# MyNiuuu/MOFA-Video

Measured on AMD Instinct MI355X. Metric: denoised frames/sec, 25f 576x1024 SVD+MOFA, 25 steps, higher is better.
Workload: dtype f16; 1 GPU; MOFA-Video-Traj, 25-frame 576x1024, 25 denoise steps + temporal VAE decode (chunk 8), single trajectory hint, SVD-XT UNet + MOFA-Adapter, CFG 1->3, seeded random weights in the reference checkpoint layout; num_frames=25, height=576, width=1024, num_inference_steps=25, decode_chunk_size=8, parallelism=1 GPU, graph_steps=False, output_finite=True

## Files before the change

include/mofa_hip.h:

```cpp
#ifndef MOFA_HIP_H
#define MOFA_HIP_H

#include <stdint.h>

#ifdef __cplusplus
extern "C" {
#endif

typedef void* mofa_stream_t;

#define MOFA_OK 0
#define MOFA_EINVAL (-22)
#define MOFA_ELAUNCH (-5)

int mofa_version(void);

enum { MOFA_MODE_PLAIN = 0, MOFA_MODE_CONV3X3 = 1, MOFA_MODE_CONVT3 = 2 };
enum { MOFA_ACT_NONE = 0, MOFA_ACT_SILU = 1, MOFA_ACT_GEGLU_PAIR = 2, MOFA_ACT_RELU = 3,
       MOFA_ACT_GELU = 4  };

typedef struct mofa_igemm_args {
    const void* x;
    const void* w;
    const float* bias;
// ... 40 lines not shown
int mofa_gn_nparts(int HW, int C);
int mofa_gn_partial_f16(const void* x, float* part, int nframes, int HW, int C, int ldx, mofa_stream_t stream);
int mofa_gn_partial_from_stats(const float* stats, float* part, int nframes, int HW, int C, mofa_stream_t stream);
int mofa_gn_finalize(const float* part, const float* gamma, const float* beta, float* scale, float* shift,
                     int nframes, int HW, int C, int frames_per_stat, float eps, mofa_stream_t stream);
int mofa_gn_reduce(const float* part, double* sums, int nframes, int HW, int C, int frames_per_stat, mofa_stream_t stream);
int mofa_gn_finalize_sums(const double* sums, const float* gamma, const float* beta, float* scale, float* shift,
                          int nframes, int C, int frames_per_stat, double count_per_group, float eps,
                          mofa_stream_t stream);
int mofa_gn_apply_f16(const void* x, const float* part, const float* gamma, const float* beta, void* y,
                      int nframes, int HW, int C, int ldx, int ldy, int frames_per_stat, float eps, int silu,
                      mofa_stream_t stream);
int mofa_gn_apply_gathered_f16(const void* x, const float* part_all, int nentries, double count_per_group,
                               const float* gamma, const float* beta, void* y, int nframes, int HW, int C,
                               int ldx, int ldy, float eps, int silu, mofa_stream_t stream);
int mofa_affine_act_f16(const void* x, const float* scale, const float* shift, void* y,
                        int nframes, int HW, int C, int ldx, int ldy, int silu, mofa_stream_t stream);
int mofa_layernorm_f16(const void* x, const float* gamma, const float* beta, void* y, int M, int C,
                       int ldx, int ldy, float eps, const float* rowvec, int rv_div, int rv_mod,
                       mofa_stream_t stream);

typedef struct mofa_ff320_args {
    const void* x;
    const float* pos;
    const void* w1p;
    const float* b1;
    const void* w2p;
    const float* b2;
    const void* r2;
    void* out;
    void* out_ln;
    const float* ln_gamma;
    const float* ln_beta;
    int32_t M, ldx, ldo, ldr2, ldoln, HW, T;
    float eps, s_acc, s1, s2, ln_eps;
    int32_t reserved[4];
} mofa_ff320_args;
int mofa_ff320_f16(const mofa_ff320_args* a, mofa_stream_t stream);

typedef struct mofa_lin320_args {
    const void* x;
    const void* wp;
    const float* bias;
    const float* rowvec;
    const void* r1;
    void* out;
    int32_t M, N, ldx, ldo, ldr1, norm;
    int32_t rv_div, rv_mul, rv_mod_in, rv_mod_out;
    float eps, s_acc, s1;
    int32_t reserved[3];
} mofa_lin320_args;
int mofa_lin320_f16(const mofa_lin320_args* a, mofa_stream_t stream);

int mofa_axpby_f32(const float* x, float* y, int64_t n, float a, float b, mofa_stream_t stream);
int mofa_resize_nearest_f32(const float* x, float* y, int n, int H, int W, int h, int w, mofa_stream_t stream);
int mofa_mask_blend_f16(const void* a, const void* b, const float* w, void* out, int M, int C, int HW, int lda,
                        int ldb, int ldo, mofa_stream_t stream);
int mofa_matting_blend_f16(const void* warped, const void* matting, const void* logit, void* out, float* mask_out,
                           int M, int C, int ldw, int ldm, int ldl, int ldo, mofa_stream_t stream);
int mofa_subsample_tokens_f16(const void* x, void* y, int n, int H, int W, int s, int C, int ldx, int ldy,
                              mofa_stream_t stream);
int mofa_axpby_f16(const void* x, void* y, int M, int C, int ldx, int ldy, float a, float b, mofa_stream_t stream);
int mofa_axpby_out_f16(const void* x, const void* y, void* out, int M, int C, int ldx, int ldy, int ldo, float a, float b,
                       mofa_stream_t stream);
int mofa_geglu_f16(const void* x, void* out, int M, int Ch, int ldx, int ldo, mofa_stream_t stream);
int mofa_copy2d_f16(const void* src, void* dst, int M, int C, int lds, int ldd, mofa_stream_t stream);
int mofa_silu_f32(const float* x, float* y, int n, mofa_stream_t stream);
int mofa_cast_f32_to_f16(const float* x, void* y, int64_t n, mofa_stream_t stream);
int mofa_cast_f16_to_f32(const void* x, float* y, int64_t n, mofa_stream_t stream);
int mofa_nchw_f32_to_nhwc_f16(const float* x, void* y, int n, int C, int HW, int ldo, float scale,
                              mofa_stream_t stream);
int mofa_nhwc_f16_to_nchw_f32(const void* x, float* y, int n, int C, int HW, int ldx, mofa_stream_t stream);
int mofa_timestep_embedding(const float* t, float* out, int n, int dim, mofa_stream_t stream);

int64_t mofa_softsplat_ws_bytes(int nflows, int H, int W);
int mofa_softsplat_avg_f16(const void* feat, const float* flow, void* out, void* ws,
                           int nflows, int H, int W, int C, int ldf, int ldo, mofa_stream_t stream);
int mofa_softsplat_scatter_f32(const float* in, const float* flow, float* out_sum, int N, int C, int H, int W,
                               mofa_stream_t stream);
int mofa_softsplat_weight_f32(const float* in, const float* metric, float* out, int N, int C, int H, int W, int mode,
                              mofa_stream_t stream);
int mofa_softsplat_normalize_f32(const float* summed, float* out, int N, int C, int H, int W, int eps_mode, mofa_stream_t stream);
typedef struct mofa_softsplat_grad_args {
    const float* grad;
    const float* flow;
    const float* in;
    const float* metric;
    const float* inv;
    const float* glast;
    float* grad_in;
    float* grad_flow;
    float* grad_metric;
    float* partial;
    int32_t N, C, H, W, prep, slices;
    int32_t reserved[4];
} mofa_softsplat_grad_args;
int mofa_softsplat_norm_f32(const float* flow, float* norm, void* ws, int N, int H, int W, mofa_stream_t stream);
int mofa_softsplat_grad_prologue_f32(const float* grad, const float* out, const float* norm, float* inv, float* glast,
                                     int N, int C, int H, int W, int eps_mode, mofa_stream_t stream);
int mofa_softsplat_grad_f32(const mofa_softsplat_grad_args* a, mofa_stream_t stream);
typedef struct mofa_softsplat_gather_args {
    const float* in;
    const float* flow;
    const float* metric;
    float* out;
    float* norm;
// ... 48 lines not shown
```

mofa_video_amd/_build.py:

```python
import os
import subprocess
from concurrent.futures import ThreadPoolExecutor

HERE = os.path.dirname(os.path.abspath(__file__))
CSRC = os.path.join(HERE, "csrc")
LIB = os.path.join(HERE, "libmofa_hip.so")
PROBE_LIB = os.path.join(HERE, "..", "tools", "libmofa_hip_probe.so")
SOURCES = ["igemm.hip", "igemm8.hip", "igemm320.hip", "ff320.hip", "lin320.hip", "attention.hip", "norm.hip", "elementwise.hip", "softsplat.hip", "output.hip",
           "cmp_ops.hip", "frontend.hip"]
HEADERS = [os.path.join(CSRC, "common.h"), os.path.join(CSRC, "igemm_common.h"), os.path.join(CSRC, "igemm_pipe.h"),
           os.path.join(HERE, "..", "include", "mofa_hip.h")]
FLAGS = ["--offload-arch=gfx950", "-O3", "-std=c++17", "-fPIC"]


def _hipcc():
    hipcc = os.environ.get("HIPCC", "/opt/rocm/bin/hipcc")
    return hipcc if os.path.exists(hipcc) else "hipcc"


def build(force=False, verbose=False, probe=False, variant=None, defines=()):
    objdir = os.path.join(HERE, "build", variant or ("probe" if probe else "lib"))
    os.makedirs(objdir, exist_ok=True)
    lib = os.path.join(HERE, "..", "tools", f"libmofa_hip_{variant}.so") if variant else (PROBE_LIB if probe else LIB)
    hdr_t = max(os.path.getmtime(h) for h in HEADERS if os.path.exists(h))
    flags = FLAGS + (["-DMOFA_PROBE"] if probe else []) + [f"-D{d}" for d in defines]
    jobs = []
    for s in SOURCES:
        src, obj = os.path.join(CSRC, s), os.path.join(objdir, s.replace(".hip", ".o"))
        if force or not os.path.exists(obj) or os.path.getmtime(obj) < max(os.path.getmtime(src), hdr_t):
            jobs.append([_hipcc(), *flags, "-c", src, "-o", obj])
    if not jobs and os.path.exists(lib) and all(os.path.getmtime(lib) >= os.path.getmtime(os.path.join(objdir, s.replace(".hip", ".o")))
                                                for s in SOURCES):
        return lib

    def run(cmd):
        if verbose:
            print(" ".join(cmd), flush=True)
        subprocess.run(cmd, check=True)
    with ThreadPoolExecutor(max_workers=min(len(jobs), os.cpu_count() or 4) or 1) as ex:
        list(ex.map(run, jobs))
    run([_hipcc(), "--offload-arch=gfx950", "-shared", "-fPIC", *[os.path.join(objdir, s.replace(".hip", ".o")) for s in SOURCES],
         "-o", lib])
    return lib


if __name__ == "__main__":
    import sys
    var = sys.argv[sys.argv.index("--variant") + 1] if "--variant" in sys.argv else None
    print(build(force="--incremental" not in sys.argv, verbose=True, probe="--probe" in sys.argv, variant=var,
                defines=[a[2:] for a in sys.argv if a.startswith("-D")]))
```

mofa_video_amd/blocks.py:

```python
import math

import torch

from . import lib as L
from . import ops
from .weights import (f32, interleave_geglu, pack_conv3d_t3, pack_conv3x3, pack_ff320, pack_lin320, pack_linear, pad_rows)

BIG = 1 << 30


class Sub:

    def __init__(self, sd, prefix="", device="cuda"):
        self.sd, self.prefix, self.device = sd, prefix, device

    def sub(self, name):
        return Sub(self.sd, f"{self.prefix}{name}.", self.device)

    def has(self, name):
        return f"{self.prefix}{name}" in self.sd

    def get(self, name):
        return self.sd[f"{self.prefix}{name}"].detach()

    def dev(self, t):
        return t.to(self.device)


class Ctx:

    def __init__(self, B, T):
        self.B, self.T = B, T
        self.N = B * T
        self.temb_act = None
        self.temb_all = None
        self.ctx16 = None
        self.cache = {}
        self.time_context_hw_major = True
        self.par = None
        self.ctx16_all = None
        self.half = 0
        self.halves = None


class Linear:
    def __init__(self, s, pad_n=False):
        w = s.get("weight")
        w = w.reshape(w.shape[0], -1)
        self.n_real = w.shape[0]
        b = s.get("bias") if s.has("bias") else None
        if pad_n:
            w = pad_rows(w)
            b = pad_rows(b) if b is not None else None
        self.w = s.dev(pack_linear(w))
        self.b = s.dev(f32(b)) if b is not None else None

    def __call__(self, x, **kw):
        return ops.igemm(x, self.w, self.b, **kw)

# ... 171 lines not shown
            return self.tconv2(g, T, HW, s_acc=1.0 - self.alpha, r1=xs, s1=1.0, stats=out_stats, out=out)
        assert c.B == 1
        g = _sharded_norm_convt3(self.tnorm1, self.tconv1, xs, c, HW,
                                 **(tvec(self.ttemb, self.ttemb_off) if self.ttemb is not None else {}))
        return _sharded_norm_convt3(self.tnorm2, self.tconv2, g, c, HW, s_acc=1.0 - self.alpha, r1=xs, s1=1.0, out=out)


def _sharded_norm_convt3(norm, conv, x, c, HW, r1=None, out=None, **epi):
    par, T = c.par, c.T
    M, Cc = T * HW, x.shape[1]
    nparts = ops.gn_nparts(HW, Cc)
    buf, own = par.part_buffer(nparts, x.device)
    ops.gn_partial_into(x, own, T, HW)
    halo = par.halo_begin(x, HW)
    par.gather_partials(buf, nparts)
    cnt = float(par.T_full) * HW * (Cc // 32)
    ext = torch.empty(((T + 2) * HW, Cc), dtype=x.dtype, device=x.device)
    ops.gn_apply_gathered(x, buf, cnt, norm.g, norm.b, norm.eps, ext[HW:(T + 1) * HW], T, HW, silu=True)
    if out is None:
        out = torch.empty((M, conv.w.shape[0]), dtype=x.dtype, device=x.device)
    geom = ops.convt3_geom(0, HW)

    def launch(f0, f1):
        rr = r1[f0 * HW:f1 * HW] if r1 is not None else None
        ops.igemm(ext[(f0 + 1) * HW:], conv.w, conv.b, geom=geom, M=(f1 - f0) * HW, out=out[f0 * HW:f1 * HW], r1=rr, **epi)
    split = par.split_convs and T >= 4
    if split:
        launch(1, T - 1)
    fp, fn = halo.wait()
    for src, dst in ((fp, ext[:HW]), (fn, ext[(T + 1) * HW:])):
        if src is None:
            dst.zero_()
        else:
            ops.gn_apply_gathered(src, buf, cnt, norm.g, norm.b, norm.eps, dst, 1, HW, silu=True)
    if split:
        launch(0, 1)
        launch(T - 1, T)
    else:
        launch(0, T)
    return out


class CrossAttnVec:

    def __init__(self, s):
        self.to_v = Linear(s.sub("to_v"))
        self.to_out = Linear(s.sub("to_out.0"))

    def __call__(self, ctx16):
        return ops.cast_f16_to_f32(self.to_out(self.to_v(ctx16)))


class SelfAttn:
    def __init__(self, s, heads, fold_q_scale=False, norm=None, norm_eps=1e-5):
        wq = s.get("to_q.weight")
        self.heads = heads
        self.C = wq.shape[0]
        self.head_dim = self.C // heads
        assert self.head_dim in (64, 128), f"unsupported head dim {self.head_dim}"
        self.q_prescaled = bool(fold_q_scale)
        if fold_q_scale:
            wq = (wq.float() * (self.head_dim ** -0.5 * ops.Q_FOLD_LOG2E)).to(wq.dtype)
        w = torch.cat([wq, s.get("to_k.weight"), s.get("to_v.weight")], 0)
        self.wqkv = s.dev(pack_linear(w))
        self.to_out = Linear(s.sub("to_out.0"))
        self.qkv_pk = None
        if norm is not None and self.C == 320:
            wp, bp = pack_lin320(w, None, norm.get("weight"), norm.get("bias"))
            self.qkv_pk = (s.dev(wp), s.dev(bp), norm_eps)

    def qkv_normed(self, x):
        wp, bp, eps = self.qkv_pk
        qkv = ops.lin320(x, wp, bp, norm=True, eps=eps)
        Cc = self.C
        return qkv[:, :Cc], qkv[:, Cc:2 * Cc], qkv[:, 2 * Cc:]

    @property
    def can_fuse_norm(self):
        return self.qkv_pk is not None and ops.LIN320

    def qkv(self, x):
        qkv = ops.igemm(x, self.wqkv)
        Cc = self.C
        return qkv[:, :Cc], qkv[:, Cc:2 * Cc], qkv[:, 2 * Cc:]

    def kv_into(self, x, out):
        return ops.igemm(x, self.wqkv[self.C:], out=out)

    def q(self, x):
        return ops.igemm(x, self.wqkv[:self.C])


class TransformerSpatioTemporal:
    _uid = 0

    def __init__(self, s, heads):
        TransformerSpatioTemporal._uid += 1
        self.uid = TransformerSpatioTemporal._uid
        self.heads = heads
        self.norm = GroupNorm(s.sub("norm"), 1e-6)
        self.proj_in, self.proj_out = Linear(s.sub("proj_in")), Linear(s.sub("proj_out"))
        b = s.sub("transformer_blocks.0")
        self.norm1, self.norm3 = LayerNorm(b.sub("norm1")), LayerNorm(b.sub("norm3"))
        self.attn1, self.attn2, self.ff = (SelfAttn(b.sub("attn1"), heads, fold_q_scale=True, norm=b.sub("norm1")), CrossAttnVec(b.sub("attn2")),
                                           GegluFF(b.sub("ff"), norm=b.sub("norm3")))
        t = s.sub("temporal_transformer_blocks.0")
        self.norm_in, self.tnorm1, self.tnorm3 = LayerNorm(t.sub("norm_in")), LayerNorm(t.sub("norm1")), LayerNorm(t.sub("norm3"))
        self.ff_in, self.tattn1, self.tattn2, self.tff = (GegluFF(t.sub("ff_in"), norm=t.sub("norm_in")), SelfAttn(t.sub("attn1"), heads),
                                                          CrossAttnVec(t.sub("attn2")), GegluFF(t.sub("ff"), norm=t.sub("norm3")))
        self.pos1, self.pos2 = Linear(s.sub("time_pos_embed.linear_1")), Linear(s.sub("time_pos_embed.linear_2"))
        self.alpha = _sigmoid(s.get("time_mixer.mix_factor").reshape(-1)[0])
        self.C = self.proj_in.w.shape[1]

    def _invariants(self, c):
        key = ("xf", self.uid)
        if key not in c.cache:
            dev = self.proj_in.w.device
            f0 = c.par.f0 if c.par is not None else 0
            tpos = ops.timestep_embedding(torch.arange(f0, f0 + c.T, dtype=torch.float32, device=dev), self.C)
            e = self.pos2(self.pos1(ops.cast_f32_to_f16(tpos), act=L.ACT_SILU))
            v_tm = self.tattn2(c.ctx16_all if c.ctx16_all is not None else c.ctx16)
            c.cache[key] = (self.attn2(c.ctx16), v_tm, ops.cast_f16_to_f32(e))
        return c.cache[key]

    def __call__(self, x, c, H, W, out_stats=False, out=None):
        HW, N, T, B = H * W, c.N, c.T, c.B
        v_sp, v_tm, pos = self._invariants(c)
        h = self.norm(x, N, HW)
        h = self.proj_in(h)
        fuse_qkv = self.attn1.can_fuse_norm and ops.lin320_fits(h.shape[0], 3 * self.C)
        q, k, v = self.attn1.qkv_normed(h) if fuse_qkv else self.attn1.qkv(self.norm1(h))
        a = ops.attn_spatial(q, k, v, N, self.heads, HW, head_dim=self.attn1.head_dim, prescaled=self.attn1.q_prescaled)
        h = self.attn1.to_out(a, r1=h, s1=1.0, rowvec=v_sp, rv=(T * HW, 1, 1, BIG))
        h = self.ff.fused(h) if self.ff.can_fuse else self.ff(self.norm3(h), r1=h, s1=1.0)
        pos_rv = (HW, 1, 1, T)
        fn = None
        if self.ff_in.can_fuse:
            f_own = None
            if c.par is not None and c.par.kv_slots <= 32 and c.par.kv_inplace and c.par.gather_hidden:
                hid, f_own = c.par.kv_buffer(HW, self.C, h.device)
            f, fn = self.ff_in.fused(h, pos=pos, HW=HW, T=T, ln_out=(self.tnorm1.g, self.tnorm1.b, f_own), ln_eps=self.tnorm1.eps)
        else:
            f = self.ff_in(self.norm_in(h, rowvec=pos, rv_div=HW, rv_mod=T), r1=h, s1=1.0, rowvec=pos, rv=pos_rv)
        if c.par is None:
            q, k, v = self.tattn1.qkv(fn if fn is not None else self.tnorm1(f))
            a = ops.attn_temporal(q, k, v, B, T, HW, self.heads, head_dim=self.tattn1.head_dim)
        else:
            Cc, par = self.C, c.par
            if par.kv_slots <= 32 and par.kv_inplace and par.gather_hidden:
                if fn is None:
                    hid, own = par.kv_buffer(HW, Cc, f.device)
                    fn = self.tnorm1(f, out=own)
                work = par.kv_gather_begin(hid, HW)
                q = self.tattn1.q(fn)
                work.wait()
                kv = ops.igemm(hid, self.tattn1.wqkv[Cc:])
                a = ops.attn_temporal(q, kv[:, :Cc], kv[:, Cc:], 1, par.kv_slots, HW, self.heads,
                                      head_dim=self.tattn1.head_dim, Tq=T, key_mask=par.kv_mask)
            elif par.kv_slots <= 32 and par.kv_inplace:
                fn = fn if fn is not None else self.tnorm1(f)
                kv, own = par.kv_buffer(HW, 2 * Cc, fn.device)
                self.tattn1.kv_into(fn, own)
                work = par.kv_gather_begin(kv, HW)
                q = self.tattn1.q(fn)
                work.wait()
                a = ops.attn_temporal(q, kv[:, :Cc], kv[:, Cc:], 1, par.kv_slots, HW, self.heads,
                                      head_dim=self.tattn1.head_dim, Tq=T, key_mask=par.kv_mask)
            else:
                fn = fn if fn is not None else self.tnorm1(f)
                q, k, v = self.tattn1.qkv(fn)
                kv = torch.empty((q.shape[0], 2 * Cc), dtype=torch.float16, device=q.device)
                ops.copy2d(k, kv[:, :Cc])
                ops.copy2d(v, kv[:, Cc:])
                kv = par.gather_frames(kv, HW)
                a = ops.attn_temporal(q, kv[:, :Cc], kv[:, Cc:], 1, par.T_full, HW, self.heads,
                                      head_dim=self.tattn1.head_dim, Tq=T)
        Bg = v_tm.shape[0]
        if not c.time_context_hw_major:
            quirk, tab = (T * HW, 1, 1, BIG), (v_tm if Bg == B else v_tm[c.half:c.half + B].contiguous())
        elif Bg == B:
            quirk, tab = (T * HW, HW, HW, B), v_tm
        else:
            rot = (c.half * HW) % Bg
            tab = torch.cat([v_tm[rot:], v_tm[:rot]], 0).contiguous() if rot else v_tm
            quirk = (T * HW, 0, HW, Bg)
        f = self.tattn1.to_out(a, r1=f, s1=1.0, rowvec=tab, rv=quirk)
        al = self.alpha
        if self.tff.can_fuse:
            m = self.tff.fused(f, s_acc=1.0 - al, s1=1.0 - al, r2=h, s2=al)
        else:
            m = self.tff(self.tnorm3(f), s_acc=1.0 - al, r1=f, s1=1.0 - al, r2=h, s2=al)
        return self.proj_out(m, r1=x, s1=1.0, stats=out_stats, out=out)


class DownBlock:
    def __init__(self, s, num_layers, heads, cross, downsample):
        eps = 1e-6 if cross else 1e-5
        self.resnets = [SpatioTemporalResBlock(s.sub(f"resnets.{i}"), eps) for i in range(num_layers)]
        self.attns = [TransformerSpatioTemporal(s.sub(f"attentions.{i}"), heads) for i in range(num_layers)] if cross else None
# ... 92 lines not shown
```

mofa_video_amd/lib.py:

```python
import ctypes as C
import os

import torch

_HERE = os.path.dirname(os.path.abspath(__file__))
LIB_PATH = os.environ.get("MOFA_HIP_LIB") or os.path.join(_HERE, "libmofa_hip.so")

MODE_PLAIN, MODE_CONV3X3, MODE_CONVT3 = 0, 1, 2
ACT_NONE, ACT_SILU, ACT_GEGLU_PAIR, ACT_RELU, ACT_GELU = 0, 1, 2, 3, 4
PAD_SAME, PAD_TRAILING = 0, 1
TILE_AUTO, TILE_128X128, TILE_192X128, TILE_256X256, TILE_256X320 = 0, 2, 4, 5, 6


class IgemmArgs(C.Structure):
    _fields_ = [
        ("x", C.c_void_p), ("w", C.c_void_p), ("bias", C.c_void_p), ("rowvec", C.c_void_p),
        ("r1", C.c_void_p), ("r2", C.c_void_p), ("out", C.c_void_p),
        ("M", C.c_int32), ("N", C.c_int32), ("Cin", C.c_int32),
        ("ldx", C.c_int32), ("ldo", C.c_int32), ("ldr1", C.c_int32), ("ldr2", C.c_int32),
        ("mode", C.c_int32),
        ("Hin", C.c_int32), ("Win", C.c_int32), ("Hout", C.c_int32), ("Wout", C.c_int32),
        ("stride", C.c_int32), ("up", C.c_int32), ("ksize", C.c_int32),
        ("T", C.c_int32), ("HW", C.c_int32),
        ("rv_div", C.c_int32), ("rv_mul", C.c_int32), ("rv_mod_in", C.c_int32), ("rv_mod_out", C.c_int32),
        ("act", C.c_int32),
        ("s_acc", C.c_float), ("s1", C.c_float), ("s2", C.c_float),
        ("dil", C.c_int32), ("pad", C.c_int32), ("tile", C.c_int32),
        ("workspace", C.c_void_p), ("workspace_bytes", C.c_int64),
        ("stats", C.c_void_p),
    ]


class Ff320Args(C.Structure):
    _fields_ = [
        ("x", C.c_void_p), ("pos", C.c_void_p), ("w1p", C.c_void_p), ("b1", C.c_void_p), ("w2p", C.c_void_p), ("b2", C.c_void_p),
        ("r2", C.c_void_p), ("out", C.c_void_p), ("out_ln", C.c_void_p), ("ln_gamma", C.c_void_p), ("ln_beta", C.c_void_p),
        ("M", C.c_int32), ("ldx", C.c_int32), ("ldo", C.c_int32), ("ldr2", C.c_int32), ("ldoln", C.c_int32),
        ("HW", C.c_int32), ("T", C.c_int32),
        ("eps", C.c_float), ("s_acc", C.c_float), ("s1", C.c_float), ("s2", C.c_float), ("ln_eps", C.c_float),
        ("reserved", C.c_int32 * 4),
    ]


class Lin320Args(C.Structure):
    _fields_ = [
        ("x", C.c_void_p), ("wp", C.c_void_p), ("bias", C.c_void_p), ("rowvec", C.c_void_p), ("r1", C.c_void_p), ("out", C.c_void_p),
        ("M", C.c_int32), ("N", C.c_int32), ("ldx", C.c_int32), ("ldo", C.c_int32), ("ldr1", C.c_int32), ("norm", C.c_int32),
        ("rv_div", C.c_int32), ("rv_mul", C.c_int32), ("rv_mod_in", C.c_int32), ("rv_mod_out", C.c_int32),
        ("eps", C.c_float), ("s_acc", C.c_float), ("s1", C.c_float),
        ("reserved", C.c_int32 * 3),
    ]


class SoftsplatGradArgs(C.Structure):
    _fields_ = [
        ("grad", C.c_void_p), ("flow", C.c_void_p), ("inp", C.c_void_p), ("metric", C.c_void_p), ("inv", C.c_void_p),
        ("glast", C.c_void_p), ("grad_in", C.c_void_p), ("grad_flow", C.c_void_p), ("grad_metric", C.c_void_p),
        ("partial", C.c_void_p),
        ("N", C.c_int32), ("C", C.c_int32), ("H", C.c_int32), ("W", C.c_int32), ("prep", C.c_int32), ("slices", C.c_int32),
        ("reserved", C.c_int32 * 4),
    ]


class SoftsplatGatherArgs(C.Structure):
    _fields_ = [
        ("inp", C.c_void_p), ("flow", C.c_void_p), ("metric", C.c_void_p), ("out", C.c_void_p), ("norm", C.c_void_p), ("ws", C.c_void_p),
        ("N", C.c_int32), ("C", C.c_int32), ("H", C.c_int32), ("W", C.c_int32), ("prep", C.c_int32), ("normalize", C.c_int32),
        ("eps_mode", C.c_int32), ("slices", C.c_int32),
        ("reserved", C.c_int32 * 4),
    ]


_P, _I, _F, _L = C.c_void_p, C.c_int, C.c_float, C.c_int64

PROTOTYPES = {
    "mofa_version": [],
    "mofa_igemm_f16": [_P, _P],
    "mofa_igemm_stats_ok": [_P],
    "mofa_ff320_f16": [_P, _P],
    "mofa_lin320_f16": [_P, _P],
    "mofa_attn_spatial_f16": [_P, _P, _P, _P, _I, _I, _I, _I, _I, _I, _I, _I, _F, _P],
    "mofa_attn_spatial_qb_f16": [_P, _P, _P, _P, _I, _I, _I, _I, _I, _I, _I, _I, _F, _I, _P],
    "mofa_transpose_v_f16": [_P, _P, _I, _I, _I, _I, _P],
    "mofa_attn_temporal_f16": [_P, _P, _P, _P, _I, _I, _I, _I, _I, _I, _I, _I, _I, _F, _P],
    "mofa_attn_temporal_masked_f16": [_P, _P, _P, _P, _I, _I, _I, _I, _I, _I, _I, _I, _I, _F, C.c_uint32, _P],
    "mofa_softmax_rows_f16": [_P, _I, _I, _I, _P],
    "mofa_gn_nparts": [_I, _I],
    "mofa_gn_partial_f16": [_P, _P, _I, _I, _I, _I, _P],
    "mofa_gn_partial_from_stats": [_P, _P, _I, _I, _I, _P],
    "mofa_gn_finalize": [_P, _P, _P, _P, _P, _I, _I, _I, _I, _F, _P],
    "mofa_gn_reduce": [_P, _P, _I, _I, _I, _I, _P],
    "mofa_gn_finalize_sums": [_P, _P, _P, _P, _P, _I, _I, _I, C.c_double, _F, _P],
    "mofa_gn_apply_f16": [_P, _P, _P, _P, _P, _I, _I, _I, _I, _I, _I, _F, _I, _P],
    "mofa_gn_apply_gathered_f16": [_P, _P, _I, C.c_double, _P, _P, _P, _I, _I, _I, _I, _I, _F, _I, _P],
    "mofa_affine_act_f16": [_P, _P, _P, _P, _I, _I, _I, _I, _I, _I, _P],
    "mofa_layernorm_f16": [_P, _P, _P, _P, _I, _I, _I, _I, _F, _P, _I, _I, _P],
    "mofa_axpby_f32": [_P, _P, _L, _F, _F, _P],
    "mofa_resize_nearest_f32": [_P, _P, _I, _I, _I, _I, _I, _P],
    "mofa_mask_blend_f16": [_P, _P, _P, _P, _I, _I, _I, _I, _I, _I, _P],
    "mofa_matting_blend_f16": [_P, _P, _P, _P, _P, _I, _I, _I, _I, _I, _I, _P],
    "mofa_subsample_tokens_f16": [_P, _P, _I, _I, _I, _I, _I, _I, _I, _P],
    "mofa_axpby_f16": [_P, _P, _I, _I, _I, _I, _F, _F, _P],
    "mofa_axpby_out_f16": [_P, _P, _P, _I, _I, _I, _I, _I, _F, _F, _P],
    "mofa_geglu_f16": [_P, _P, _I, _I, _I, _I, _P],
    "mofa_copy2d_f16": [_P, _P, _I, _I, _I, _I, _P],
    "mofa_silu_f32": [_P, _P, _I, _P],
    "mofa_cast_f32_to_f16": [_P, _P, _L, _P],
    "mofa_cast_f16_to_f32": [_P, _P, _L, _P],
    "mofa_nchw_f32_to_nhwc_f16": [_P, _P, _I, _I, _I, _I, _F, _P],
    "mofa_nhwc_f16_to_nchw_f32": [_P, _P, _I, _I, _I, _I, _P],
    "mofa_timestep_embedding": [_P, _P, _I, _I, _P],
    "mofa_softsplat_ws_bytes": [_I, _I, _I],
    "mofa_softsplat_avg_f16": [_P, _P, _P, _P, _I, _I, _I, _I, _I, _I, _P],
    "mofa_softsplat_scatter_f32": [_P, _P, _P, _I, _I, _I, _I, _P],
    "mofa_softsplat_weight_f32": [_P, _P, _P, _I, _I, _I, _I, _I, _P],
    "mofa_softsplat_normalize_f32": [_P, _P, _I, _I, _I, _I, _I, _P],
    "mofa_softsplat_norm_f32": [_P, _P, _P, _I, _I, _I, _P],
    "mofa_softsplat_grad_prologue_f32": [_P, _P, _P, _P, _P, _I, _I, _I, _I, _I, _P],
    "mofa_softsplat_grad_f32": [_P, _P],
    "mofa_softsplat_gather_f32": [_P, _P],
    "mofa_flow_downscale_f32": [_P, _P, _I, _I, _I, _I, _P],
    "mofa_prepare_model_input": [_P, _P, _P, _I, _I, _I, _F, _P],
    "mofa_cfg_euler_step": [_P, _P, _I, _I, _I, _F, _F, _F, _F, _P],
    "mofa_prepare_model_input_dev": [_P, _P, _P, _I, _I, _I, _P, _P],
    "mofa_cfg_euler_step_dev": [_P, _P, _I, _I, _I, _P, _F, _F, _P],
    "mofa_step_select": [_P, _P, _P, _I, _P],
    "mofa_pool2d_f16": [_P, _P, _I, _I, _I, _I, _I, _I, _I, _I, _I, _I, _P],
    "mofa_resize_bilinear_ac_f16": [_P, _P, _I, _I, _I, _I, _I, _I, _I, _I, _P],
    "mofa_resize_bilinear_ac_f32": [_P, _P, _I, _I, _I, _I, _I, _P],
    "mofa_flow_expectation_f16": [_P, _P, _I, _I, _I, _I, _F, _P],
    "mofa_filter1d_reflect_f32": [_P, _P, _P, _I, _I, _I, _I, _I, _P],
    "mofa_resize_bicubic_ac_f32": [_P, _P, _I, _I, _I, _I, _I, _P],
    "mofa_patchify_f16": [_P, _P, _I, _I, _I, _I, _I, _I, _P],
# ... 42 lines not shown
```

mofa_video_amd/ops.py:

```python
import ctypes as C
import struct
import threading

import torch

from . import lib as L

F16 = torch.float16
F32 = torch.float32


class LaunchTimer:

    def __init__(self):
        self.rec = []
        self.tags = []

    def start(self):
        e = torch.cuda.Event(enable_timing=True)
        e.record()
        return e

    def stop(self, name, e0, flops=0.0, nbytes=0.0, tag=None):
        e1 = torch.cuda.Event(enable_timing=True)
        e1.record()
        self.rec.append((name, e0, e1, flops, nbytes))
        if tag is not None:
            self.tags.append((tag, len(self.rec) - 1))

    def by_tag(self):
        torch.cuda.synchronize()
        out = {}
        for tag, i in self.tags:
            _, e0, e1, fl, _ = self.rec[i]
            d = out.setdefault(tag, [0, 0.0, 0.0])
            d[0] += 1
            d[1] += e0.elapsed_time(e1) * 1e-3
            d[2] += fl
        return out

    def summary(self):
        torch.cuda.synchronize()
        out = {}
        for name, e0, e1, fl, nb in self.rec:
            d = out.setdefault(name, dict(launches=0, seconds=0.0, flops=0.0, bytes=0.0))
            d["launches"] += 1
            d["seconds"] += e0.elapsed_time(e1) * 1e-3
            d["flops"] += fl
            d["bytes"] += nb
        return out


TIMER = None
# ... 250 lines not shown
        _written(yl)
    args = _FF320_ARGS.pack(x.data_ptr(), L.ptr(pos) or 0, w1p.data_ptr(), b1.data_ptr(), w2p.data_ptr(), b2.data_ptr(),
                            L.ptr(r2) or 0, out.data_ptr(), L.ptr(yl) or 0, L.ptr(pg) or 0, L.ptr(pb) or 0,
                            M, _ld(x), _ld(out), _ld(r2) if r2 is not None else 0, _ld(yl) if yl is not None else 0, HW, T,
                            eps, s_acc, s1, s2 if r2 is not None else 0.0, ln_eps, 0, 0, 0, 0)
    t0 = TIMER.start() if TIMER is not None else None
    rc = lib.mofa_ff320_f16(args, L.stream_ptr())
    if rc != 0:
        L.check(rc, "mofa_ff320_f16")
    if t0 is not None:
        TIMER.stop("igemm_f16_kernel", t0, flops=2.0 * M * (2560 * 320 + 320 * 1280), tag=(9, 0, 0, M, 320, 320, 0))
    return out if ln_out is None else (out, yl)


_LIN320_ARGS = struct.Struct("@6P10i3f3i")
assert _LIN320_ARGS.size == C.sizeof(L.Lin320Args)
LIN320 = True


def lin320_fits(M, ldo):
    return (M + 256) * ldo * 2 < 0xFFFFFFFF


def lin320(x, wp, bias=None, norm=False, eps=1e-5, rowvec=None, rv=(1, 1, 1, 1 << 30), r1=None, s1=1.0, s_acc=1.0, out=None):
    lib = L.load()
    _chk(x, F16)
    M, N = x.shape[0], wp.shape[0] * 64
    assert x.shape[1] == 320 and wp.dtype is F16 and wp.numel() == N * 320
    if out is None:
        out = torch.empty((M, N), dtype=F16, device=x.device)
    else:
        assert out.dtype is F16 and out.shape[0] == M and out.shape[1] >= N
        _written(out)
    if bias is not None:
        assert bias.dtype is F32 and bias.numel() == N
    if rowvec is not None:
        assert rowvec.dtype is F32 and rowvec.dim() == 2 and rowvec.shape[1] == N and rowvec.stride(1) == 1
        assert rowvec.is_contiguous() or (rowvec.stride(0) % N == 0 and rv[1] == rowvec.stride(0) // N), (rowvec.stride(), N, rv)
    if r1 is not None:
        assert r1.dtype is F16 and r1.shape[0] == M and r1.shape[1] >= N
    args = _LIN320_ARGS.pack(x.data_ptr(), wp.data_ptr(), L.ptr(bias) or 0, L.ptr(rowvec) or 0, L.ptr(r1) or 0, out.data_ptr(),
                             M, N, _ld(x), _ld(out), _ld(r1) if r1 is not None else 0, 1 if norm else 0,
                             rv[0], rv[1], rv[2], rv[3], eps, s_acc, s1, 0, 0, 0)
    t0 = TIMER.start() if TIMER is not None else None
    rc = lib.mofa_lin320_f16(args, L.stream_ptr())
    if rc != 0:
        L.check(rc, "mofa_lin320_f16")
    if t0 is not None:
        TIMER.stop("igemm_f16_kernel", t0, flops=2.0 * M * N * 320, tag=(10, 0, 0, M, N, 320, 0))
    return out


Q_FOLD_LOG2E = 1.4426950408889634


def attn_spatial(q, k, v, nframes, heads, S, head_dim=64, scale=None, out=None, prescaled=False, query_blocks=0):
    lib = L.load()
    Cc = heads * head_dim
    scale = -1.0 if prescaled else (head_dim ** -0.5 if scale is None else scale)
    st = L.stream_ptr()
    if out is None:
        out = torch.empty((nframes * S, Cc), dtype=F16, device=q.device)
    else:
        _written(out)
    t0 = TIMER.start() if TIMER is not None else None
    L.check(lib.mofa_attn_spatial_qb_f16(L.ptr(q), L.ptr(k), L.ptr(v), L.ptr(out), nframes, heads, head_dim, S, _ld(q),
                                         _ld(k), _ld(v), _ld(out), scale, int(query_blocks), st), "mofa_attn_spatial_qb_f16")
    if t0 is not None:
        TIMER.stop("attn_spatial_kernel", t0, flops=4.0 * S * S * Cc * nframes)
    return out


def attn_temporal(q, k, v, nclips, T, HW, heads, head_dim=64, scale=None, out=None, Tq=None, key_mask=None):
    lib = L.load()
    assert _ld(k) == _ld(v)
    Tq = T if Tq is None else Tq
    scale = head_dim ** -0.5 if scale is None else scale
    if out is None:
        out = torch.empty((nclips * Tq * HW, heads * head_dim), dtype=F16, device=q.device)
    else:
        _written(out)
    if key_mask is None:
        L.check(lib.mofa_attn_temporal_f16(L.ptr(q), L.ptr(k), L.ptr(v), L.ptr(out), nclips, Tq, T, HW, heads, head_dim,
                                           _ld(q), _ld(k), _ld(out), scale, L.stream_ptr()), "mofa_attn_temporal_f16")
    else:
        L.check(lib.mofa_attn_temporal_masked_f16(L.ptr(q), L.ptr(k), L.ptr(v), L.ptr(out), nclips, Tq, T, HW, heads, head_dim,
                                                  _ld(q), _ld(k), _ld(out), scale, int(key_mask), L.stream_ptr()),
                "mofa_attn_temporal_masked_f16")
    return out


def softmax_rows_(x):
    lib = L.load()
    L.check(lib.mofa_softmax_rows_f16(L.ptr(x), x.shape[0], x.shape[1], _ld(x), L.stream_ptr()), "mofa_softmax_rows_f16")
    return x


def transpose_v(v, nframes, ncb, S):
    lib = L.load()
    vt = torch.empty((nframes * ncb * 64, S), dtype=F16, device=v.device)
    L.check(lib.mofa_transpose_v_f16(L.ptr(v), L.ptr(vt), nframes, ncb, S, _ld(v), L.stream_ptr()),
            "mofa_transpose_v_f16")
    return vt


def axpby_(x, y, a=1.0, b=1.0):
# ... 443 lines not shown
```

mofa_video_amd/weights.py:

```python
import torch

KPAD = 64


def _pad_cin(w, dim):
    cin = w.shape[dim]
    pad = (-cin) % KPAD
    if pad == 0:
        return w
    shape = list(w.shape)
    shape[dim] = pad
    return torch.cat([w, w.new_zeros(shape)], dim=dim)


def pack_linear(w):
    w = w.reshape(w.shape[0], -1)
    return _pad_cin(w, 1).to(torch.float16).contiguous()


def pack_conv3x3(w):
    w = _pad_cin(w, 1)
    n, cin, kh, kw = w.shape
    return w.permute(0, 2, 3, 1).reshape(n, kh * kw * cin).to(torch.float16).contiguous()

# ... 8 lines not shown
    pad = (-w.shape[0]) % mult
    if pad == 0:
        return w
    return torch.cat([w, w.new_zeros((pad,) + tuple(w.shape[1:]))], dim=0)


def interleave_geglu(w, b):
    n2 = w.shape[0]
    ch = n2 // 2
    assert ch % 16 == 0
    idx = torch.arange(n2).reshape(2, ch // 16, 16).permute(1, 0, 2).reshape(-1)
    return w[idx].contiguous(), (b[idx].contiguous() if b is not None else None)


def pack_ff320(w1, b1, w2, gamma, beta):
    C, H = 320, 1280
    w1, w2 = w1.detach().float().cpu().reshape(2 * H, C), w2.detach().float().cpu().reshape(C, H)
    gamma, beta = gamma.detach().float().cpu(), beta.detach().float().cpu()
    b1f = (b1.detach().float().cpu() if b1 is not None else torch.zeros(2 * H)) + w1 @ beta
    w1g = (w1 * gamma[None, :]).to(torch.float16)
    lane = torch.arange(64)
    n, lh = lane % 32, lane // 32
    c, t, s_, e = torch.arange(40), torch.arange(2), torch.arange(20), torch.arange(8)
    rows = (t[None, :, None, None, None] * H + 32 * c[:, None, None, None, None] + n[None, None, None, :, None])
    cols = 16 * s_[None, None, :, None, None] + 8 * lh[None, None, None, :, None] + e[None, None, None, None, :]
    w1p = w1g[rows.expand(40, 2, 20, 64, 8), cols.expand(40, 2, 20, 64, 8)].contiguous()
    j, u, jj = torch.arange(10), torch.arange(2), torch.arange(8)
    rows2 = 32 * j[None, :, None, None, None] + n[None, None, None, :, None]
    cols2 = (32 * c[:, None, None, None, None] + 16 * u[None, None, :, None, None] + 4 * lh[None, None, None, :, None] +
             (jj & 3)[None, None, None, None, :] + 8 * (jj >> 2)[None, None, None, None, :])
    w2p = w2.to(torch.float16)[rows2.expand(40, 10, 2, 64, 8), cols2.expand(40, 10, 2, 64, 8)].contiguous()
    return w1p, b1f.contiguous(), w2p


def pack_lin320(w, b=None, gamma=None, beta=None):
    w = w.detach().float().cpu().reshape(w.shape[0], -1)
    N, K = w.shape
    assert K == 320 and N % 64 == 0, (N, K)
    bias = b.detach().float().cpu().clone() if b is not None else None
    if beta is not None:
        bias = (bias if bias is not None else torch.zeros(N)) + w @ beta.detach().float().cpu()
    if gamma is not None:
        w = w * gamma.detach().float().cpu()[None, :]
    wh = w.to(torch.float16)
    lane = torch.arange(64)
    n, lh = lane % 32, lane // 32
    c, t, s_, e = torch.arange(N // 64), torch.arange(2), torch.arange(20), torch.arange(8)
    rows = 64 * c[:, None, None, None, None] + 32 * t[None, :, None, None, None] + n[None, None, None, :, None]
    cols = 16 * s_[None, None, :, None, None] + 8 * lh[None, None, None, :, None] + e[None, None, None, None, :]
    shp = (N // 64, 2, 20, 64, 8)
    return wh[rows.expand(shp), cols.expand(shp)].contiguous(), (bias.contiguous() if bias is not None else None)


def f32(t):
    return t.detach().to(torch.float32).contiguous()
```

Baseline: 4.197 frames/s.

## Fuse QKV projection and temporal attention into one kernel for C=320

Adds a HIP kernel that, for the 320-channel temporal self-attention, computes per-head Q, K and V projections with MFMA from weights streamed into LDS, runs softmax attention over the T frames in registers, and writes the output directly. It replaces the separate QKV GEMM and temporal attention launch, so the QKV intermediate never goes through global memory. Weights are repacked per head (q,k,v interleaved) at load time, and the kernel is persistent with a rotating three-slot DMA buffer. It is only used for C=320, 5 heads, T<=32, and is on by default but can be disabled through an environment variable.

```diff
diff --git a/include/mofa_hip.h b/include/mofa_hip.h
--- a/include/mofa_hip.h
+++ b/include/mofa_hip.h
@@ -116,6 +116,16 @@
 } mofa_lin320_args;
 int mofa_lin320_f16(const mofa_lin320_args* a, mofa_stream_t stream);
 
+typedef struct mofa_tattn320_args {
+    const void* x;
+    const void* wp;
+    void* out;
+    int32_t nclips, T, HW, ldx, ldo;
+    float scale;
+    int32_t reserved[4];
+} mofa_tattn320_args;
+int mofa_tattn320_f16(const mofa_tattn320_args* a, mofa_stream_t stream);
+
 int mofa_axpby_f32(const float* x, float* y, int64_t n, float a, float b, mofa_stream_t stream);
 int mofa_resize_nearest_f32(const float* x, float* y, int n, int H, int W, int h, int w, mofa_stream_t stream);
 int mofa_mask_blend_f16(const void* a, const void* b, const float* w, void* out, int M, int C, int HW, int lda,
diff --git a/mofa_video_amd/_build.py b/mofa_video_amd/_build.py
--- a/mofa_video_amd/_build.py
+++ b/mofa_video_amd/_build.py
@@ -6,7 +6,7 @@
 CSRC = os.path.join(HERE, "csrc")
 LIB = os.path.join(HERE, "libmofa_hip.so")
 PROBE_LIB = os.path.join(HERE, "..", "tools", "libmofa_hip_probe.so")
-SOURCES = ["igemm.hip", "igemm8.hip", "igemm320.hip", "ff320.hip", "lin320.hip", "attention.hip", "norm.hip", "elementwise.hip", "softsplat.hip", "output.hip",
+SOURCES = ["igemm.hip", "igemm8.hip", "igemm320.hip", "ff320.hip", "lin320.hip", "tattn320.hip", "attention.hip", "norm.hip", "elementwise.hip", "softsplat.hip", "output.hip",
            "cmp_ops.hip", "frontend.hip"]
 HEADERS = [os.path.join(CSRC, "common.h"), os.path.join(CSRC, "igemm_common.h"), os.path.join(CSRC, "igemm_pipe.h"),
            os.path.join(HERE, "..", "include", "mofa_hip.h")]
diff --git a/mofa_video_amd/blocks.py b/mofa_video_amd/blocks.py
--- a/mofa_video_amd/blocks.py
+++ b/mofa_video_amd/blocks.py
@@ -4,7 +4,7 @@
 
 from . import lib as L
 from . import ops
-from .weights import (f32, interleave_geglu, pack_conv3d_t3, pack_conv3x3, pack_ff320, pack_lin320, pack_linear, pad_rows)
+from .weights import (f32, interleave_geglu, pack_conv3d_t3, pack_conv3x3, pack_ff320, pack_lin320, pack_linear, pack_tattn320, pad_rows)
 
 BIG = 1 << 30
 
@@ -282,7 +282,7 @@
 
 
 class SelfAttn:
-    def __init__(self, s, heads, fold_q_scale=False, norm=None, norm_eps=1e-5):
+    def __init__(self, s, heads, fold_q_scale=False, norm=None, norm_eps=1e-5, temporal=False):
         wq = s.get("to_q.weight")
         self.heads = heads
         self.C = wq.shape[0]
@@ -298,6 +298,9 @@
         if norm is not None and self.C == 320:
             wp, bp = pack_lin320(w, None, norm.get("weight"), norm.get("bias"))
             self.qkv_pk = (s.dev(wp), s.dev(bp), norm_eps)
+        self.tattn_pk = None
+        if temporal and self.C == 320 and heads == 5 and not fold_q_scale:
+            self.tattn_pk = s.dev(pack_tattn320(wq, s.get("to_k.weight"), s.get("to_v.weight"), heads))
 
     def qkv_normed(self, x):
         wp, bp, eps = self.qkv_pk
@@ -336,7 +339,7 @@
                                            GegluFF(b.sub("ff"), norm=b.sub("norm3")))
         t = s.sub("temporal_transformer_blocks.0")
         self.norm_in, self.tnorm1, self.tnorm3 = LayerNorm(t.sub("norm_in")), LayerNorm(t.sub("norm1")), LayerNorm(t.sub("norm3"))
-        self.ff_in, self.tattn1, self.tattn2, self.tff = (GegluFF(t.sub("ff_in"), norm=t.sub("norm_in")), SelfAttn(t.sub("attn1"), heads),
+        self.ff_in, self.tattn1, self.tattn2, self.tff = (GegluFF(t.sub("ff_in"), norm=t.sub("norm_in")), SelfAttn(t.sub("attn1"), heads, temporal=True),
                                                           CrossAttnVec(t.sub("attn2")), GegluFF(t.sub("ff"), norm=t.sub("norm3")))
         self.pos1, self.pos2 = Linear(s.sub("time_pos_embed.linear_1")), Linear(s.sub("time_pos_embed.linear_2"))
         self.alpha = _sigmoid(s.get("time_mixer.mix_factor").reshape(-1)[0])
@@ -373,8 +376,12 @@
         else:
             f = self.ff_in(self.norm_in(h, rowvec=pos, rv_div=HW, rv_mod=T), r1=h, s1=1.0, rowvec=pos, rv=pos_rv)
         if c.par is None:
-            q, k, v = self.tattn1.qkv(fn if fn is not None else self.tnorm1(f))
-            a = ops.attn_temporal(q, k, v, B, T, HW, self.heads, head_dim=self.tattn1.head_dim)
+            src = fn if fn is not None else self.tnorm1(f)
+            if ops.TATTN320 and self.tattn1.tattn_pk is not None and ops.tattn320_fits(src, B, T, HW, self.C):
+                a = ops.tattn320(src, self.tattn1.tattn_pk, B, T, HW, heads=self.heads)
+            else:
+                q, k, v = self.tattn1.qkv(src)
+                a = ops.attn_temporal(q, k, v, B, T, HW, self.heads, head_dim=self.tattn1.head_dim)
         else:
             Cc, par = self.C, c.par
             if par.kv_slots <= 32 and par.kv_inplace and par.gather_hidden:
diff --git a/mofa_video_amd/csrc/tattn320.hip b/mofa_video_amd/csrc/tattn320.hip
--- /dev/null
+++ b/mofa_video_amd/csrc/tattn320.hip
@@ -0,0 +1,221 @@
+#include "common.h"
+
+namespace {
+
+constexpr int TA_KS = 20, TA_CHUNK = 2 * TA_KS * 1024;
+constexpr int TA_NCHUNK = 15;
+constexpr int TA_OFF_T = 3 * TA_CHUNK;
+constexpr int TA_LDS_BYTES = TA_OFF_T + 8 * 4096;
+constexpr int TA_LOOK = 6;
+constexpr unsigned TA_OOB = 0xF0000000u;
+
+typedef unsigned u32x2 __attribute__((ext_vector_type(2)));
+typedef unsigned u32x4 __attribute__((ext_vector_type(4)));
+template <int V> struct IC { static constexpr int v = V; };
+template <int I, int N, typename F>
+__device__ __forceinline__ void static_for(F&& f) {
+    if constexpr (I < N) { f(IC<I>{}); static_for<I + 1, N>(f); }
+}
+#define TA_LDS_PTR(p) ((__attribute__((address_space(3))) void*)(p))
+
+template <int K>
+__device__ __forceinline__ void ta_barrier() {
+    asm volatile("s_waitcnt vmcnt(%0) lgkmcnt(0)\n\ts_barrier" ::"n"(K) : "memory");
+}
+
+__global__ __launch_bounds__(512, 2) void tattn320_kernel(const mofa_tattn320_args a, const int ntiles, const int nseq) {
+    extern __shared__ __attribute__((aligned(16))) char smem_ta[];
+    const int tid = threadIdx.x, lane = tid & 63;
+    const int wave = __builtin_amdgcn_readfirstlane(tid >> 6);
+    const int l31 = lane & 31, lh = lane >> 5;
+    const int T = a.T, HW = a.HW;
+    const unsigned M = (unsigned)a.nclips * (unsigned)T * (unsigned)HW;
+
+    const auto rs = __builtin_amdgcn_make_buffer_rsrc((void*)a.wp, 0, (unsigned)TA_NCHUNK * TA_CHUNK, 0x00020000);
+    const auto rsx = __builtin_amdgcn_make_buffer_rsrc((void*)a.x, 0, ((M - 1u) * (unsigned)a.ldx + 320u) * 2u, 0x00020000);
+    const auto rso = __builtin_amdgcn_make_buffer_rsrc(a.out, 0, ((M - 1u) * (unsigned)a.ldo + 320u) * 2u, 0x00020000);
+    const unsigned voff = (unsigned)lane * 16u;
+    auto dma_chunk = [&](int chunk, int slot) __attribute__((always_inline)) {
+        char* dst = smem_ta + slot * TA_CHUNK + wave * 5120;
+        const int src = chunk * TA_CHUNK + wave * 5120;
+        __builtin_amdgcn_raw_ptr_buffer_load_lds(rs, TA_LDS_PTR(dst), 16, voff, src, 0, 0);
+        __builtin_amdgcn_raw_ptr_buffer_load_lds(rs, TA_LDS_PTR(dst), 16, voff, src, 1024, 0);
+        __builtin_amdgcn_raw_ptr_buffer_load_lds(rs, TA_LDS_PTR(dst), 16, voff, src, 2048, 0);
+        __builtin_amdgcn_raw_ptr_buffer_load_lds(rs, TA_LDS_PTR(dst), 16, voff, src, 3072, 0);
+        __builtin_amdgcn_raw_ptr_buffer_load_lds(rs, TA_LDS_PTR(dst + 4096), 16, voff, src + 4096, 0, 0);
+    };
+    const char* wl = smem_ta + lane * 16;
+    const unsigned ldx2 = (unsigned)a.ldx * 2u, ldo2 = (unsigned)a.ldo * 2u;
+    auto x_off = [&](int tile) __attribute__((always_inline)) -> unsigned {
+        const int seq = tile * 8 + wave;
+        const int b = seq / HW, p = seq - b * HW;
+        return (seq < nseq && l31 < T) ? (unsigned)((b * T + l31) * HW + p) * ldx2 + 16u * (unsigned)lh : TA_OOB;
+    };
+    auto x_load = [&](unsigned off, int s) __attribute__((always_inline)) -> f16x8 {
+        return __builtin_bit_cast(f16x8, __builtin_amdgcn_raw_buffer_load_b128(rsx, off + 32u * (unsigned)s, 0, 0));
+    };
+    const float qscale = a.scale * 1.4426950408889634f;
+
+    dma_chunk(0, 0);
+    dma_chunk(1, 1);
+    asm volatile("s_waitcnt vmcnt(0)" ::: "memory");
+    f16x8 xf[TA_KS];
+    {
+        const unsigned xo = x_off((int)blockIdx.x);
+#pragma unroll
+        for (int s = 0; s < TA_KS; ++s) xf[s] = x_load(xo, s);
+    }
+    int cnext = 2;
+    auto chunk_mfma = [&](auto slot_c, auto swap_c, f32x16 (&acc)[2], const bool reload, const unsigned xo_next) __attribute__((always_inline)) {
+        constexpr int SLOT = decltype(slot_c)::v;
+        constexpr bool SWAP = decltype(swap_c)::v != 0;
+        const char* w = wl + SLOT * TA_CHUNK;
+        auto frag = [&](int i) __attribute__((always_inline)) -> f16x8 {
+            return *(const f16x8*)(w + ((i & 1) * TA_KS + (i >> 1)) * 1024);
+        };
+        constexpr int RING = TA_LOOK + 2;
+        f16x8 ring[RING];
+#pragma unroll
+        for (int t = 0; t < 2; ++t)
+#pragma unroll
+            for (int r = 0; r < 16; ++r) acc[t][r] = 0.f;
+#pragma unroll
+        for (int i = 0; i < TA_LOOK; ++i) ring[i] = frag(i);
+        static_for<0, 2 * TA_KS>([&](auto ic) __attribute__((always_inline)) {
+            constexpr int i = decltype(ic)::v;
+            if constexpr ((i & 1) == 0) {
+                if constexpr (i + TA_LOOK + 1 < 2 * TA_KS) ring[(i + TA_LOOK + 1) % RING] = frag(i + TA_LOOK + 1);
+                if constexpr (i + TA_LOOK < 2 * TA_KS) ring[(i + TA_LOOK) % RING] = frag(i + TA_LOOK);
+            }
+            if constexpr (SWAP) {
+                acc[i & 1] = __builtin_amdgcn_mfma_f32_32x32x16_f16(xf[i >> 1], ring[i % RING], acc[i & 1], 0, 0, 0);
+                if constexpr (i & 1) {
+                    if (reload) xf[i >> 1] = x_load(xo_next, i >> 1);
+                }
+            } else {
+                acc[i & 1] = __builtin_amdgcn_mfma_f32_32x32x16_f16(ring[i % RING], xf[i >> 1], acc[i & 1], 0, 0, 0);
+            }
+        });
+    };
+    auto next_dma = [&](int slot) __attribute__((always_inline)) {
+        dma_chunk(cnext, slot);
+        cnext = cnext + 1 == TA_NCHUNK ? 0 : cnext + 1;
+    };
+    auto round16 = [&](const f32x16& v, const float m, f16x8 (&o)[2]) __attribute__((always_inline)) {
+#pragma unroll
+        for (int r = 0; r < 16; ++r) o[r >> 3][r & 7] = (f16)(v[r] * m);
+    };
+
+    for (int tile = blockIdx.x; tile < ntiles; tile += gridDim.x) {
+        const bool more = tile + (int)gridDim.x < ntiles;
+        const unsigned xo_next = more ? x_off(tile + (int)gridDim.x) : TA_OOB;
+        const int seq = tile * 8 + wave;
+        const int b = seq / HW, p = seq - b * HW;
+        const int f0 = lane >> 3;
+        const unsigned obase = (unsigned)((b * T + f0) * HW + p) * ldo2 + 16u * (unsigned)(lane & 7);
+        const unsigned ostep = 8u * (unsigned)HW * ldo2;
+        const bool sok = seq < nseq;
+
+        for (int h = 0; h < 5; ++h) {
+            f32x16 acc[2];
+            f16x8 qh[2][2], kh[2][2], pf[2];
+            ta_barrier<9>();
+            next_dma(2);
+            chunk_mfma(IC<0>{}, IC<0>{}, acc, false, 0u);
+            round16(acc[0], qscale, qh[0]);
+            round16(acc[1], qscale, qh[1]);
+            ta_barrier<9>();
+            next_dma(0);
+            chunk_mfma(IC<1>{}, IC<0>{}, acc, false, 0u);
+            round16(acc[0], 1.0f, kh[0]);
+            round16(acc[1], 1.0f, kh[1]);
+            float inv;
+            {
+                f32x16 s;
+#pragma unroll
+                for (int r = 0; r < 16; ++r) s[r] = 0.f;
+#pragma unroll
+                for (int t = 0; t < 2; ++t)
+#pragma unroll
+                    for (int u = 0; u < 2; ++u) s = __builtin_amdgcn_mfma_f32_32x32x16_f16(kh[t][u], qh[t][u], s, 0, 0, 0);
+                float mx = -1e30f;
+#pragma unroll
+                for (int r = 0; r < 16; ++r) {
+                    const int key = (r & 3) + 8 * (r >> 2) + 4 * lh;
+                    if (key >= T) s[r] = -1e30f;
+                    mx = fmaxf(mx, s[r]);
+                }
+                mx = fmaxf(mx, __shfl_xor(mx, 32, 64));
+                float sum = 0.f;
+#pragma unroll
+                for (int r = 0; r < 16; ++r) {
+                    const float pr = __builtin_amdgcn_exp2f(s[r] - mx);
+                    sum += pr;
+                    pf[r >> 3][r & 7] = (f16)pr;
+                }
+                sum += __shfl_xor(sum, 32, 64);
+                inv = 1.0f / sum;
+            }
+            ta_barrier<5>();
+            next_dma(1);
+            chunk_mfma(IC<2>{}, IC<1>{}, acc, more && h == 4, xo_next);
+            f16x8 vh[2][2];
+            round16(acc[0], 1.0f, vh[0]);
+            round16(acc[1], 1.0f, vh[1]);
+#pragma unroll
+            for (int t = 0; t < 2; ++t) {
+#pragma unroll
+                for (int r = 0; r < 16; ++r) acc[t][r] = 0.f;
+#pragma unroll
+                for (int u = 0; u < 2; ++u) acc[t] = __builtin_amdgcn_mfma_f32_32x32x16_f16(vh[t][u], pf[u], acc[t], 0, 0, 0);
+            }
+            char* ts = smem_ta + TA_OFF_T + wave * 4096;
+#pragma unroll
+            for (int t = 0; t < 2; ++t) {
+                f16x4 gq[4];
+#pragma unroll
+                for (int q = 0; q < 4; ++q)
+#pragma unroll
+                    for (int e = 0; e < 4; ++e) gq[q][e] = (f16)(acc[t][4 * q + e] * inv);
+#pragma unroll
+                for (int k = 0; k < 2; ++k) {
+                    const u32x2 a2 = __builtin_bit_cast(u32x2, gq[2 * k]), b2 = __builtin_bit_cast(u32x2, gq[2 * k + 1]);
+                    const auto rx = __builtin_amdgcn_permlane32_swap(a2[0], b2[0], false, false);
+                    const auto ry = __builtin_amdgcn_permlane32_swap(a2[1], b2[1], false, false);
+                    const u32x4 vv = {rx[0], ry[0], rx[1], ry[1]};
+                    const int seg = 4 * t + 2 * k + lh;
+                    *(u32x4*)(ts + l31 * 128 + ((seg ^ (l31 & 7)) * 16)) = vv;
+                }
+            }
+            asm volatile("s_waitcnt lgkmcnt(0)" ::: "memory");
+#pragma unroll
+            for (int i = 0; i < 4; ++i) {
+                const int r = f0 + 8 * i;
+                const u32x4 o = *(const u32x4*)(ts + r * 128 + (((lane & 7) ^ (r & 7)) * 16));
+                const unsigned off = (sok && r < T) ? obase + (unsigned)i * ostep + 128u * (unsigned)h : TA_OOB;
+                __builtin_amdgcn_raw_buffer_store_b128(o, rso, off, 0, 0);
+            }
+        }
+    }
+    asm volatile("s_waitcnt vmcnt(0)" ::: "memory");
+}
+
+}
+
+extern "C" int mofa_tattn320_f16(const mofa_tattn320_args* a, mofa_stream_t stream) {
+    if (!a || !a->x || !a->wp || !a->out || a->nclips <= 0 || a->HW <= 0 || a->T < 1 || a->T > 32) return MOFA_EINVAL;
+    if ((a->ldx & 7) || (a->ldo & 7) || a->ldx < 320 || a->ldo < 320 || (((size_t)a->x) & 15) || (((size_t)a->out) & 15) || (((size_t)a->wp) & 15))
+        return MOFA_EINVAL;
+    if (!(a->scale > 0.f)) return MOFA_EINVAL;
+    if (a->reserved[0] || a->reserved[1] || a->reserved[2] || a->reserved[3]) return MOFA_EINVAL;
+    const long long nseq = (long long)a->nclips * a->HW, M = nseq * a->T;
+    if (nseq + 8 >= 0x7fffffffLL / 8 || M * a->ldx * 2 >= (long long)TA_OOB || M * a->ldo * 2 >= (long long)TA_OOB) return MOFA_EINVAL;
+    static LaunchSetup setup;
+    const int n_cu = setup.cus([](int) { return mofa_lds_optin((const void*)tattn320_kernel, TA_LDS_BYTES); });
+    if (n_cu == 0) return MOFA_ELAUNCH;
+    const int ntiles = (int)((nseq + 7) / 8);
+    const int grid = ntiles < n_cu ? ntiles : n_cu;
+    hipLaunchKernelGGL(tattn320_kernel, dim3(grid), dim3(512), TA_LDS_BYTES, (hipStream_t)stream, *a, ntiles, (int)nseq);
+    MOFA_CHECK_LAUNCH();
+    return MOFA_OK;
+}
diff --git a/mofa_video_amd/lib.py b/mofa_video_amd/lib.py
--- a/mofa_video_amd/lib.py
+++ b/mofa_video_amd/lib.py
@@ -52,6 +52,15 @@
     ]
 
 
+class Tattn320Args(C.Structure):
+    _fields_ = [
+        ("x", C.c_void_p), ("wp", C.c_void_p), ("out", C.c_void_p),
+        ("nclips", C.c_int32), ("T", C.c_int32), ("HW", C.c_int32), ("ldx", C.c_int32), ("ldo", C.c_int32),
+        ("scale", C.c_float),
+        ("reserved", C.c_int32 * 4),
+    ]
+
+
 class SoftsplatGradArgs(C.Structure):
     _fields_ = [
         ("grad", C.c_void_p), ("flow", C.c_void_p), ("inp", C.c_void_p), ("metric", C.c_void_p), ("inv", C.c_void_p),
@@ -79,6 +88,7 @@
     "mofa_igemm_stats_ok": [_P],
     "mofa_ff320_f16": [_P, _P],
     "mofa_lin320_f16": [_P, _P],
+    "mofa_tattn320_f16": [_P, _P],
     "mofa_attn_spatial_f16": [_P, _P, _P, _P, _I, _I, _I, _I, _I, _I, _I, _I, _F, _P],
     "mofa_attn_spatial_qb_f16": [_P, _P, _P, _P, _I, _I, _I, _I, _I, _I, _I, _I, _F, _I, _P],
     "mofa_transpose_v_f16": [_P, _P, _I, _I, _I, _I, _P],
diff --git a/mofa_video_amd/ops.py b/mofa_video_amd/ops.py
--- a/mofa_video_amd/ops.py
+++ b/mofa_video_amd/ops.py
@@ -1,4 +1,5 @@
 import ctypes as C
+import os
 import struct
 import threading
 
@@ -355,6 +356,37 @@
 
 
 Q_FOLD_LOG2E = 1.4426950408889634
+
+_TATTN320_ARGS = struct.Struct("@3P5if4i")
+assert _TATTN320_ARGS.size == C.sizeof(L.Tattn320Args)
+TATTN320 = os.environ.get("MOFA_TATTN320", "1") != "0"
+_TATTN320_LIMIT = 0xF0000000
+
+
+def tattn320_fits(x, nclips, T, HW, ldo):
+    M = nclips * T * HW
+    return bool(x.is_cuda and 1 <= T <= 32 and M * _ld(x) * 2 < _TATTN320_LIMIT and M * ldo * 2 < _TATTN320_LIMIT)
+
+
+def tattn320(x, wp, nclips, T, HW, heads=5, scale=None, out=None):
+    lib = L.load()
+    _chk(x, F16)
+    M = nclips * T * HW
+    assert heads == 5 and x.shape[0] == M and x.shape[1] == 320 and wp.dtype is F16 and wp.numel() == 960 * 320, (x.shape, wp.shape, heads)
+    scale = 64 ** -0.5 if scale is None else scale
+    if out is None:
+        out = torch.empty((M, 320), dtype=F16, device=x.device)
+    else:
+        assert out.dtype is F16 and out.is_cuda and out.shape[0] == M and out.shape[1] >= 320
+        _written(out)
+    args = _TATTN320_ARGS.pack(x.data_ptr(), wp.data_ptr(), out.data_ptr(), nclips, T, HW, _ld(x), _ld(out), scale, 0, 0, 0, 0)
+    t0 = TIMER.start() if TIMER is not None else None
+    rc = lib.mofa_tattn320_f16(args, L.stream_ptr())
+    if rc != 0:
+        L.check(rc, "mofa_tattn320_f16")
+    if t0 is not None:
+        TIMER.stop("igemm_f16_kernel", t0, flops=2.0 * M * 960 * 320 + 4.0 * M * T * 320, tag=(11, 0, 0, M, 960, 320, 0))
+    return out
 
 
 def attn_spatial(q, k, v, nframes, heads, S, head_dim=64, scale=None, out=None, prescaled=False, query_blocks=0):
diff --git a/mofa_video_amd/weights.py b/mofa_video_amd/weights.py
--- a/mofa_video_amd/weights.py
+++ b/mofa_video_amd/weights.py
@@ -84,5 +84,12 @@
     return wh[rows.expand(shp), cols.expand(shp)].contiguous(), (bias.contiguous() if bias is not None else None)
 
 
+def pack_tattn320(wq, wk, wv, heads=5):
+    ws = [w.detach().float().cpu().reshape(w.shape[0], -1) for w in (wq, wk, wv)]
+    assert all(w.shape == (64 * heads, 320) for w in ws), [tuple(w.shape) for w in ws]
+    rows = torch.cat([w[64 * h:64 * (h + 1)] for h in range(heads) for w in ws], 0)
+    return pack_lin320(rows)[0]
+
+
 def f32(t):
     return t.detach().to(torch.float32).contiguous()
```

Result: no change. 4.236 frames/s, median of 6 (+0.9%).
